# zihang-student/Codes-of-IPD-SsN-AMG-method

Measured on AMD Instinct MI355X. Metric: V-cycle throughput (DoF*cycles/sec), m=n=1024 OT grid, higher is better.
Workload: dtype f64

## Files before the change

### codes_of_ipd_ssn_amg_method_amd/csrc/ipd_resident.h

```cpp
#pragma once

#include "ipd_resident_proto.h"

static constexpr int RES_P3_LD = 1152;
static constexpr int RES_P4_LD = 2 * RES_P4_SEG + 64;

struct ResLevelDesc {
    int N, nf, S;
    const unsigned short* pci;
    const double* pva;
    const double* diag;
    const double* dinv;
    const double* Axi;
    const double* xx;
};
struct ResDesc {
    ResLevelDesc L1, L2;
    ResLevelDesc L3;
    ResCsr Pt2, P2;
    ResCsr Pt3, P3;
    ResCsr Pt4, P4;
    ResCsr A3;
    ResCsr A4;
    int three;
// ... 86 lines not shown
        s1 = __builtin_fma(a[q + 1], y[q + 1], s1);
        s2 = __builtin_fma(a[q + 2], y[q + 2], s2);
        s3 = __builtin_fma(a[q + 3], y[q + 3], s3);
    }
    return (s0 + s1) + (s2 + s3);
}

__device__ __forceinline__ double res_csr_rowdot(const ResCsr& M, int e0, int e1, int lane,
                                                 const double* sm, int off) {
    double s = 0.0;
    for (int t = e0 + lane; t < e1; t += 64 * 8) {
        int jj[8];
        double aa[8];
#pragma unroll
        for (int u = 0; u < 8; ++u) {
            const int tt = t + 64 * u;
            const int tc = tt < e1 ? tt : e0;
            jj[u] = M.ci[tc];
            aa[u] = M.va[tc];
        }
#pragma unroll
        for (int u = 0; u < 8; ++u) s += (t + 64 * u < e1) ? aa[u] * sm[off + jj[u]] : 0.0;
    }
    return wave_sum(s);
}

__device__ __forceinline__ double res_red8(const double* red) {
    double t = 0.0;
#pragma unroll
    for (int k = 0; k < RES_WAVES; ++k) t += red[k];
    return t;
}

__device__ __forceinline__ double res_red8_tree(const double* red) {
    static_assert(RES_WAVES == 8, "eight waves");
    double v[RES_WAVES];
#pragma unroll
    for (int k = 0; k < RES_WAVES; ++k) v[k] = red[k];
    return ((v[0] + v[1]) + (v[2] + v[3])) + ((v[4] + v[5]) + (v[6] + v[7]));
}

__device__ __forceinline__ void res_swap_halves32(double& a, double& b) {
    const auto lo = __builtin_amdgcn_permlane32_swap((unsigned)__double2loint(a), (unsigned)__double2loint(b), false, false);
    const auto hi = __builtin_amdgcn_permlane32_swap((unsigned)__double2hiint(a), (unsigned)__double2hiint(b), false, false);
    a = __hiloint2double((int)hi[0], (int)lo[0]);
    b = __hiloint2double((int)hi[1], (int)lo[1]);
}
__device__ __forceinline__ void res_swap_rows16(double& a, double& b) {
    const auto lo = __builtin_amdgcn_permlane16_swap((unsigned)__double2loint(a), (unsigned)__double2loint(b), false, false);
    const auto hi = __builtin_amdgcn_permlane16_swap((unsigned)__double2hiint(a), (unsigned)__double2hiint(b), false, false);
    a = __hiloint2double((int)hi[0], (int)lo[0]);
    b = __hiloint2double((int)hi[1], (int)lo[1]);
}
__device__ __forceinline__ void res_cs_rows(const double (&A)[RES_WAVES][2], double v0, double v1, double* part_out,
                                            int w, int lane) {
    static_assert(RES_WAVES == 8, "eight rows per block and workgroup");
    double p[RES_WAVES];
#pragma unroll
    for (int r = 0; r < RES_WAVES; ++r) p[r] = __builtin_fma(A[r][1], v1, A[r][0] * v0);
    double q[4];
#pragma unroll
    for (int k = 0; k < 4; ++k) {
        res_swap_halves32(p[k], p[k + 4]);
        q[k] = p[k] + p[k + 4];
    }
    double t[2];
#pragma unroll
    for (int k = 0; k < 2; ++k) {
        res_swap_rows16(q[k], q[k + 2]);
        t[k] = q[k] + q[k + 2];
    }
    const bool f = (lane & 8) != 0;
    const double keep = f ? t[1] : t[0], send = f ? t[0] : t[1];
    double u = keep + dpp_get<0x128, 0xf>(send);
    u = subwave_sum(u, 8);
    if ((lane & 7) == 0) part_out[8 * (lane >> 3) + w] = u;
}

enum res_class {
    RES_CL_HALF = 0,
    RES_CL_START = 1,
    RES_CL_RR = 2,
    RES_CL_RESTRICT = 3,
    RES_CL_LEVEL2 = 4,
    RES_CL_PROLONG = 5,
    RES_CL_TOP = 6,
    RES_NCLASS = 8
};

template <int KE1, int KE2, int KE3 = 0, bool POLY2 = false, bool DIAG = true, bool FULL = false>
__global__ __launch_bounds__(BT, 2) void k_resident(const ResDesc D, const double* __restrict__ bvec,
                                                    double* xg, double* out, int fixed_cycles) {
    static_assert(!POLY2 || (KE3 == 0 && KE1 == 16), "POLY2: three-level hierarchies in column slices (resident_takes_poly2)");
    static_assert(!FULL || POLY2, "FULL: the composed instantiation only (resident_takes_full)");
    static_assert(DIAG || KE1 == 16, "the production form exists for the column-slice kernels");
    constexpr int FG = 2 * BT / RES_WAVES;
    if constexpr (FULL) __builtin_assume(__builtin_amdgcn_workitem_id_x() < (unsigned)BT);
    constexpr bool THREE = KE3 > 0;
    constexpr bool POLY3 = KE3 == 1;
    constexpr int K3 = (THREE && !POLY3) ? KE3 : 2;
    extern __shared__ __attribute__((aligned(16))) char res_smem[];
    double* sm = reinterpret_cast<double*>(res_smem);
    const char* smb = res_smem;
    const int tid = threadIdx.x, w = tid >> 6, lane = tid & 63;
#define RES_REMOTE (FULL ? 0 : D.remote)
#define RES_WIDENT (FULL ? 1 : D.wident)
    const int b = blockIdx.x, G = FULL ? FG : gridDim.x - (RES_REMOTE ? 1 : 0);
    const int N1 = FULL ? 4 * BT : D.L1.N, N2 = FULL ? 2 * BT : D.L2.N, nf = FULL ? 2 * BT : D.L1.nf, nc = N1 - nf;
    const int Nt = FULL ? 1 : D.Nt;
    if (RES_REMOTE && b == G) {
        __shared__ PhaseLds tail_lds;
        __shared__ double tail_red[16];
        __shared__ double tail_part[48 + SOLVE_ML + 1];
        __shared__ int tail_stat[RES_WAVES];
        res_tail_workgroup(D.tail, res_smem, &tail_lds, tail_red, tail_part, tail_stat);
        return;
    }
    constexpr int oX = 0, oE1 = RES_NMAX, oE2 = 2 * RES_NMAX, oRR1 = 3 * RES_NMAX;
    constexpr int oR1 = 4 * RES_NMAX, oAX1 = 5 * RES_NMAX, oR2 = 6 * RES_NMAX, oRR2 = 7 * RES_NMAX;
    constexpr int oAX2 = 8 * RES_NMAX;
    constexpr int oRHO = 9 * RES_NMAX;
    constexpr int oBETA = oAX2 + RES_NMAX / 2;
    constexpr int oU = oRR2;
    constexpr int oR3 = 9 * RES_NMAX + RES_NMAX / 2, oE3 = oR3 + RES_TAIL_MAX, oP3 = oE3 + RES_TAIL_MAX;
    constexpr int oPART = oR3, oPART9 = oR3 + 2 * RES_WAVES * RES_WAVES;
    static_assert(2 * RES_WAVES * RES_WAVES + 2 * RES_WAVES <= 3 * RES_TAIL_MAX, "the totals fit the tail's slots");
    constexpr int oRED = oP3 + RES_TAIL_MAX;
    constexpr int oPUB = oRED + 2 * RES_WAVES;
    constexpr int oOWN = oPUB + 2 * RES_WAVES;
// ... 143 lines not shown
#define dgC sm[oOWN + 3 * RES_WAVES + w]
#define dvC sm[oOWN + 4 * RES_WAVES + w]
#define bC sm[oOWN + 5 * RES_WAVES + w]
#define dg2 sm[oOWN + 6 * RES_WAVES + w]
#define dv2 sm[oOWN + 7 * RES_WAVES + w]
#define dg3 sm[oOWN + 8 * RES_WAVES + w]
#define dv3 sm[oOWN + 9 * RES_WAVES + w]
    const bool nsp = FULL ? true : D.isnsp != 0;
    const double xx1 = nsp ? D.L1.xx[0] : 1.0, xx2 = nsp ? D.L2.xx[0] : 1.0;
    const double xx3 = (THREE && nsp) ? D.L3.xx[0] : 1.0;
    const double rxx1 = 1.0 / xx1, rxx2 = 1.0 / xx2, rxx3 = 1.0 / xx3;
    for (int j = tid; j < N1; j += BT) {
        sm[oX + j] = xg[j];
        sm[oE1 + j] = 0.0;
        sm[oAX1 + j] = D.L1.Axi[j];
    }
    for (int j = tid; j < N2; j += BT) {
        sm[oE2 + j] = 0.0;
        sm[oAX2 + j] = D.L2.Axi[j];
    }
    if (THREE)
        for (int j = tid; j < N3; j += BT) {
            sm[oE3L + j] = 0.0;
            sm[oAX3L + j] = D.L3.Axi[j];
        }
    const bool tail1 = FULL ? true : !THREE && Nt == 1 && N2 <= RES_NMAX / 2;
    constexpr int oP3C = oRR2 + RES_NMAX / 2;
    const bool lfirst = FULL ? true : D.localfirst && D.nu >= 1 && N2 <= RES_NMAX / 2 && nf <= RES_NMAX / 2;
    const bool lfirst2 = lfirst && !THREE;
    constexpr int oDV1 = oR2 + RES_NMAX / 2, oDV2 = oE2 + RES_NMAX / 2;
    if (lfirst) {
        for (int j = tid; j < nf; j += BT) sm[oDV1 + j] = D.L1.dinv[j];
        if (lfirst2)
            for (int j = tid; j < N2; j += BT) sm[oDV2 + j] = D.L2.dinv[j];
    }
    const bool xm = FULL ? true : !THREE && D.xm != 0 && nc == N2 && D.wident != 0;
    unsigned xbits = 0;
    if (xm) {
        unsigned long long wf[16], wc[16];
#pragma unroll
        for (int q = 0; q < 16; ++q) {
            wf[q] = D.xm_fbits[(size_t)rF * D.xm_nwf + (q < D.xm_nwf ? q : 0)];
            wc[q] = D.xm_cbits[(size_t)(rC - nf) * D.xm_nwc + (q < D.xm_nwc ? q : 0)];
        }
        unsigned lo = 0, hi = 0;
#pragma unroll
        for (int q = 0; q < 16; ++q) {
            lo |= (vF && q < D.xm_nwf) ? (unsigned)((wf[q] >> lane) & 1ull) << q : 0u;
            hi |= (vC && q < D.xm_nwc) ? (unsigned)((wc[q] >> lane) & 1ull) << q : 0u;
        }
        xbits = lo | (hi << 16);
        for (int j = tid; j < nf; j += BT) sm[oRHO + j] = D.xm_rho[j];
        for (int j = tid; j < nc; j += BT) sm[oBETA + j] = D.xm_beta[j];
    }
    double h33 = 0.0;
    if (tail1) {
        for (int j = tid; j < N2; j += BT) {
            double v = 0.0;
            if (POLY2) {
                v = D.p2rows[(size_t)N2 * D.p2ld + j];
            } else {
                for (int t = D.P3.rp[j]; t < D.P3.rp[j + 1]; ++t)
                    if (D.P3.ci[t] == 0) v = D.P3.va[t];
            }
            sm[oP3C + j] = v;
        }
        for (int t = D.A3.rp[0]; t < D.A3.rp[1]; ++t)
            if (D.A3.ci[t] == 0) h33 = D.A3.va[t];
    }
    if (tid == 0) *fail = 0;
    __syncthreads();

    const auto rs = __builtin_amdgcn_make_buffer_rsrc(D.gran0, 0, 2 * RES_GRAN_MAX * 16, 0x00020000);
    unsigned seq = 0;
    bool dead = false;
    const bool dbg = DIAG && D.dbg != nullptr && b == 0 && tid == 0;
#define RES_SKIPPED(sq) (DIAG && (sq) == D.dbg_skip_seq && b == G - 1)
    if (dbg) {
        dbg_acc[0] = dbg_acc[3] = dbg_acc[4] = dbg_acc[5] = dbg_acc[6] = dbg_acc[7] = dbg_acc[8] = 0;
        dbg_acc[1] = __builtin_amdgcn_s_memtime();
        dbg_acc[2] = __builtin_amdgcn_s_memrealtime();
        if constexpr (KE1 == 16)
            for (int k = 0; k < 2 * RES_NCLASS; ++k) cls_acc[k] = 0u;
    }
    auto cls_begin = [&](int c) __attribute__((always_inline)) {
        if constexpr (KE1 == 16) {
            if (dbg) __hip_atomic_fetch_sub(cls_acc + c, (unsigned)__builtin_amdgcn_s_memtime(), __ATOMIC_RELAXED, __HIP_MEMORY_SCOPE_WORKGROUP);
        }
    };
    auto cls_end = [&](int c) __attribute__((always_inline)) {
        if constexpr (KE1 == 16) {
            if (dbg) {
                __hip_atomic_fetch_add(cls_acc + c, (unsigned)__builtin_amdgcn_s_memtime(), __ATOMIC_RELAXED, __HIP_MEMORY_SCOPE_WORKGROUP);
                __hip_atomic_fetch_add(cls_acc + RES_NCLASS + c, 1u, __ATOMIC_RELAXED, __HIP_MEMORY_SCOPE_WORKGROUP);
            }
        }
    };

#define RES_HANDOFF(NJ, n, gA, cA, gB, cB, STORE, EXTRA, want_sums, t0, t1)                        \
    RES_HANDOFF_P(NJ, n, gA, cA, gB, cB, {}, STORE, EXTRA, want_sums, t0, t1)
#define RES_HANDOFF_P(NJ, n, gA, cA, gB, cB, PRE, STORE, EXTRA, want_sums, t0, t1)                 \
    RES_HANDOFF_PV(NJ, n, gA, cA, gB, cB, sm[oPUB + lane], PRE, STORE, EXTRA, want_sums, t0, t1)
#define RES_HANDOFF_PV(NJ, n, gA, cA, gB, cB, PUBV, PRE, STORE, EXTRA, want_sums, t0, t1)          \
    RES_HANDOFF_PVA(NJ, n, gA, cA, gB, cB, PUBV, PRE, STORE, {}, EXTRA, want_sums, t0, t1)
#define RES_HANDOFF_PVA(NJ, n, gA, cA, gB, cB, PUBV, PRE, STORE, AFTER, EXTRA, want_sums, t0, t1)  \
    do {                                                                                           \
// ... 12 lines not shown
            const bool second_ = lane >= RES_WAVES;                                                \
            if (lane < 2 * RES_WAVES && l8_ < (second_ ? (cB) : (cA)) &&                           \
                !RES_SKIPPED(seq))                                                                 \
                res_publish(rs, seq, (second_ ? (gB) : (gA)) + l8_, (PUBV));                       \
        }                                                                                          \
        double p0 = 0.0, p1 = 0.0;                                                                 \
        _Pragma("unroll") for (int u_ = 0; u_ < NJ; ++u_) {                                        \
            const int j = tid + u_ * BT;                                                           \
            if (j < (n)) { PRE; }                                                                  \
        }                                                                                          \
        EXTRA;                                                                                     \
        if (dbg) dbg_acc[0] -= __builtin_amdgcn_s_memtime();                                       \
        for (int ps_ = 0; ps_ < D.presleep; ++ps_) __builtin_amdgcn_s_sleep(1);                    \
        if (res_sweep<NJ>(rs, seq, (n), dead, D.tmo, hv_, D.pollsleep)) {                             \
            *fail = 1;                                                                             \
            if (lane == 0) __hip_atomic_store(D.tmo, seq, __ATOMIC_RELAXED, __HIP_MEMORY_SCOPE_AGENT); \
        }                                                                                          \
        if (dbg) {                                                                                 \
            const long long t_ = __builtin_amdgcn_s_memtime();                                     \
            dbg_acc[0] += t_;                                                                      \
            dbg_acc[4] -= t_;                                                                      \
        }                                                                                          \
        _Pragma("unroll") for (int u_ = 0; u_ < NJ; ++u_) {                                        \
            const int j = tid + u_ * BT;                                                           \
            if (j < (n)) {                                                                         \
                const double v = hv_[u_];                                                          \
                STORE;                                                                             \
            }                                                                                      \
        }                                                                                          \
        AFTER;                                                                                     \
        if (want_sums) {                                                                           \
            p0 = wave_sum(p0);                                                                     \
            if ((want_sums) > 1) p1 = wave_sum(p1);                                                \
            if (lane == 0) {                                                                       \
                red[w] = p0;                                                                       \
                if ((want_sums) > 1) red[RES_WAVES + w] = p1;                                      \
            }                                                                                      \
        }                                                                                          \
        if (dbg) {                                                                                 \
            const long long t_ = __builtin_amdgcn_s_memtime();                                     \
            dbg_acc[4] += t_;                                                                      \
            dbg_acc[5] -= t_;                                                                      \
        }                                                                                          \
        __syncthreads();                                                                           \
        if (dbg) dbg_acc[5] += __builtin_amdgcn_s_memtime();                                       \
        if (want_sums) {                                                                           \
            t0 = res_red8_tree(red);                                                               \
            if ((want_sums) > 1) t1 = res_red8_tree(red + RES_WAVES);                              \
        }                                                                                          \
    } while (0)

    auto masked_sum = [&](unsigned bits, int off, int n) __attribute__((always_inline)) {
        double s0 = 0.0, s1 = 0.0;
        (void)n;
        const double* base = sm + off + lane;
        for (int q0 = 0; q0 < 16; q0 += 8) {
            double x[8];
#pragma unroll
            for (int q = 0; q < 8; ++q) x[q] = base[64 * (q0 + q)];
            const unsigned bq = bits >> q0;
#pragma unroll
            for (int q = 0; q < 8; q += 2) {
                s0 += ((bq >> q) & 1u) ? x[q] : 0.0;
                s1 += ((bq >> (q + 1)) & 1u) ? x[q + 1] : 0.0;
            }
        }
        return wave_sum(s0 + s1);
    };
    double c1 = 0.0, c2s = 0.0;
    double sumr2p = 0.0;
    (void)sumr2p;
    const double p2ws = POLY2 ? D.p2w[N2] : 0.0;
    double dum0 = 0.0, dum1 = 0.0;
    (void)dum0;
    (void)dum1;

    int csFed = -1, csBuf = 0;
    double eFo = 0.0, eCo = 0.0;
    (void)csFed; (void)csBuf; (void)eFo; (void)eCo;
    bool topfed = false;
    (void)topfed;
    auto cs_both_rows = [&](int off) __attribute__((always_inline)) {
        const double f0 = tid < nc ? sm[off + nf + tid] : 0.0, f1 = tid + BT < nc ? sm[off + nf + tid + BT] : 0.0;
        const double g0 = tid < nf ? sm[off + tid] : 0.0, g1 = tid + BT < nf ? sm[off + tid + BT] : 0.0;
        res_cs_rows(AF, f0, f1, sm + oPART, w, lane);
        res_cs_rows(AC, g0, g1, sm + oPART + RES_WAVES * RES_WAVES, w, lane);
        csFed = -1;
        eFo = eCo = 0.0;
    };

    auto cs_row_value = [&](int off, bool rhs_b) __attribute__((always_inline)) {
        const bool sec = lane >= RES_WAVES;
        const int r = lane & (RES_WAVES - 1);
        const int row = sec ? RES_OWN_ROW(loC, hiC, r) : RES_OWN_ROW(loF, hiF, r);
        const double T = res_red8_tree(sm + oPART + RES_WAVES * lane);
        const double dg_ = sm[oOWN + (sec ? 3 : 0) * RES_WAVES + r];
        const double base = rhs_b ? sm[oOWN + (sec ? 5 : 2) * RES_WAVES + r] : sm[oR1 + row];
        return base - (T + dg_ * sm[off + row]);
    };

    auto top = [&]() __attribute__((always_inline)) {
        double nrm2 = 0.0, sumr = 0.0;
        bool fed = false;
        if constexpr (FULL) {
            if (topfed) {
                fed = true;
                topfed = false;
                ++seq;
                if (*fail) dead = true;
                double hv[4];
                if (dbg) dbg_acc[0] -= __builtin_amdgcn_s_memtime();
                for (int ps = 0; ps < D.presleep; ++ps) __builtin_amdgcn_s_sleep(1);
                if (res_sweep<4>(rs, seq, N1, dead, D.tmo, hv, D.pollsleep)) {
                    *fail = 1;
                    if (lane == 0) __hip_atomic_store(D.tmo, seq, __ATOMIC_RELAXED, __HIP_MEMORY_SCOPE_AGENT);
                }
                if (dbg) {
                    const long long t_ = __builtin_amdgcn_s_memtime();
                    dbg_acc[0] += t_;
                    dbg_acc[4] -= t_;
                }
                double p0 = 0.0, p1 = 0.0;
#pragma unroll
                for (int u = 0; u < 4; ++u) {
                    const int j = tid + u * BT;
                    const double v = hv[u];
                    sm[oR1 + j] = v;
                    sm[oE1 + j] = 0.0;
                    p0 += v * v;
                    p1 += v;
                }
                p0 = wave_sum(p0);
// ... 129 lines not shown
                    const long long t_ = __builtin_amdgcn_s_memtime();
                    dbg_acc[0] += t_;
                    dbg_acc[4] -= t_;
                }
#pragma unroll
                for (int u = 0; u < 2; ++u) {
                    const int j = blk0 + tid + u * BT;
                    const double en = hv[u] + cc;
                    sm[oE1 + j] = en;
                    if (frows) {
                        const double xn = xo[u] + en;
                        sm[oX + j] = xn;
                        mv[u] = xn;
                    } else {
                        mv[u] = en;
                    }
                }
                csBuf ^= 1;
                if (frows)
                    res_cs_rows(AC, mv[0], mv[1], sm + oPART + RES_WAVES * RES_WAVES * csBuf, w, lane);
                else
                    res_cs_rows(AF, mv[0], mv[1], sm + oPART + RES_WAVES * RES_WAVES * csBuf, w, lane);
                if (dbg) {
                    const long long t_ = __builtin_amdgcn_s_memtime();
                    dbg_acc[4] += t_;
                    dbg_acc[3] -= t_;
                }
                __syncthreads();
                if (dbg) dbg_acc[3] += __builtin_amdgcn_s_memtime();
                cls_end(RES_CL_HALF);
                cls_begin(frows ? RES_CL_TOP : RES_CL_RR);
                const double* totF = frows ? sm + oPART3 : sm + oPART + RES_WAVES * RES_WAVES * csBuf;
                const double* totC = frows ? sm + oPART + RES_WAVES * RES_WAVES * csBuf : sm + oPART3;
                if (frows) {
                    if (w == 0 && lane < 2 * RES_WAVES) {
                        const bool sec = lane >= RES_WAVES;
                        const int r = lane & (RES_WAVES - 1);
                        const int row = (sec ? loC : loF) + r;
                        const double T = res_red8_tree((sec ? totC : totF) + RES_WAVES * r);
                        const double dg_ = sm[oOWN + (sec ? 3 : 0) * RES_WAVES + r];
                        const double base = sm[oOWN + (sec ? 5 : 2) * RES_WAVES + r];
                        const double val = base - (T + dg_ * sm[oX + row]);
                        if (!RES_SKIPPED(seq + 1)) res_publish(rs, seq + 1, row, val);
                    }
                    topfed = true;
                } else {
                    if (w == 0 && lane < RES_WAVES) {
                        const double TF = res_red8_tree(totF + RES_WAVES * lane);
                        const double TC = res_red8_tree(totC + RES_WAVES * lane);
                        const double dF_ = sm[oOWN + 0 * RES_WAVES + lane], dC_ = sm[oOWN + 3 * RES_WAVES + lane];
                        const double rF_ = sm[oR1 + loF + lane], rC_ = sm[oR1 + loC + lane];
                        const double val = rF_ - (TF + dF_ * eFo);
                        if (!RES_SKIPPED(seq + 1)) res_publish(rs, seq + 1, loF + lane, val);
                        sm[oRR1 + loC + lane] = rC_ - (TC + dC_ * eCo);
                    }
                }
                csFed = -1;
                eFo = eCo = 0.0;
                return;
            }
        }
        cls_begin(start ? RES_CL_START : RES_CL_HALF);
        ++seq;
        if (*fail) dead = true;
        if (ezero && first) {
            eFo = eCo = 0.0;
            cs_finish(frows, first, true, seq);
        } else if (!FULL && csFed != me) {
            const double v0 = tid < noth ? sm[oE1 + oth0 + tid] : 0.0;
            const double v1 = tid + BT < noth ? sm[oE1 + oth0 + tid + BT] : 0.0;
            csBuf ^= 1;
            if (frows)
                res_cs_rows(AF, v0, v1, sm + oPART + RES_WAVES * RES_WAVES * csBuf, w, lane);
            else
                res_cs_rows(AC, v0, v1, sm + oPART + RES_WAVES * RES_WAVES * csBuf, w, lane);
            eFo = sm[oE1 + RES_OWN_ROW(loF, hiF, lane)];
            eCo = sm[oE1 + RES_OWN_ROW(loC, hiC, lane)];
            __syncthreads();
            cs_finish(frows, first, false, seq);
        }
        const double cc = c1;
        double pa[2] = {0.0, 0.0}, pb[2] = {0.0, 0.0}, p0 = 0.0;
        if (!first) {
#pragma unroll
            for (int u = 0; u < 2; ++u) {
                const int j = tid + u * BT;
                if (j < nblk) {
                    pa[u] = sm[oR1 + blk0 + j];
                    pb[u] = sm[oAX1 + blk0 + j];
                }
            }
            for (int jo = tid; jo < noth; jo += BT) {
                const double en = sm[oE1 + oth0 + jo] + cc;
                sm[oE1 + oth0 + jo] = en;
                p0 += sm[oR1 + oth0 + jo] - sm[oAX1 + oth0 + jo] * en;
            }
        }
        if (dbg) dbg_acc[0] -= __builtin_amdgcn_s_memtime();
        for (int ps = 0; ps < D.presleep; ++ps) __builtin_amdgcn_s_sleep(1);
        double hv[2] = {0.0, 0.0};
        if (res_sweep<2>(rs, seq, nblk, dead, D.tmo, hv, D.pollsleep)) {
            *fail = 1;
            if (lane == 0) __hip_atomic_store(D.tmo, seq, __ATOMIC_RELAXED, __HIP_MEMORY_SCOPE_AGENT);
        }
        if (dbg) {
            const long long t_ = __builtin_amdgcn_s_memtime();
            dbg_acc[0] += t_;
// ... 387 lines not shown
            {
                const double s = wave_sum(res_rowdot<K3, 8 * oE3L>(c3, a3, smb)) + dg3 * sm[oE3L + r3];
                if (lane == 0) sm[oPUB + w] = sm[oR3L + r3] - s;
                RES_HANDOFF3({ sm[oRR3L + j] = v; }, 0, dum0);
            }
            if (RES_REMOTE)
                remote_tail(D.Pt4, oRR3L, oE3L, oR3L, oAX3L, xx3, N3, c3s);
            else
                local_tail(D.Pt4, D.A4, D.P4, oRR3L, oE3L, oR3L, oAX3L, xx3, N3, c3s);
            for (int s = 0; s < nu; ++s) sweep3(false);
        }
    };

    auto visit2 = [&](bool keep) __attribute__((always_inline)) {
        const int nu = D.nu;
        for (int s = (lfirst2 && !keep) ? 1 : 0; s < nu; ++s) sweep2(!keep && s == 0);
        {
            cls_begin(RES_CL_LEVEL2);
            const double s = wave_sum(res_rowdot_fma<KE2, 8 * oE2>(c2, a2, smb)) + dg2 * sm[oE2 + r2];
            if (lane == 0) sm[oPUB + w] = sm[oR2 + r2] - s;
            RES_HANDOFF(4, N2, lo2, hi2 - lo2, 0, 0, { sm[oRR2 + j] = v; }, {}, 0, dum0, dum1);
        }
        if (dbg) dbg_acc[7] -= __builtin_amdgcn_s_memtime();
        if (THREE) {
            {
                const double s = res_csr_rowdot(D.Pt3, rowp[12 * w + 8], rowp[12 * w + 9], lane, sm, oRR2);
                if (lane == 0) sm[oPUB + w] = s;
                double sumr = 0.0;
                RES_HANDOFF3({ sm[oR3L + j] = v; sm[oE3L + j] = 0.0; p0 += v; }, (nsp ? 1 : 0), sumr);
                c3s = nsp ? sumr * rxx3 : 0.0;
                sumr3 = sumr;
            }
            for (int leg = 0; leg < (D.wcycle ? 2 : 1); ++leg) visit3(leg == 1);
            {
                const double sP = res_csr_rowdot(D.P3, rowp[12 * w + 10], rowp[12 * w + 11], lane, sm, oE3L);
                if (lane == 0) sm[oPUB + w] = sm[oE2 + r2] + sP;
                double xig = 0.0;
                RES_HANDOFF_P(4, N2, lo2, hi2 - lo2, 0, 0, { pa_[u_] = sm[oR2 + j]; pb_[u_] = sm[oAX2 + j]; },
                              { sm[oE2 + j] = v; p0 += pa_[u_] - pb_[u_] * v; }, {}, (nsp ? 1 : 0), xig, dum1);
                c2s = nsp ? xig * rxx2 : 0.0;
            }
        } else {
            tail();
        }
        if (dbg) dbg_acc[7] += __builtin_amdgcn_s_memtime();
        cls_end(RES_CL_LEVEL2);
        for (int s = 0; s < nu; ++s) sweep2(false);
    };

    auto poly2_fed = [&]() __attribute__((always_inline)) {
        if constexpr (POLY2) {
            ++seq;
            if (*fail) dead = true;
            if (dbg) dbg_acc[3] -= __builtin_amdgcn_s_memtime();
            __syncthreads();
            if (dbg) dbg_acc[3] += __builtin_amdgcn_s_memtime();
            const bool pub = w == 0 && lane < RES_WAVES && lane < hi2 - lo2;
            if (pub && !RES_SKIPPED(seq)) res_publish(rs, seq, lo2 + lane, sm[oPUB + lane]);
            const double s0 = tid < N2 ? sm[oP3C + tid] : 0.0, s1 = tid + BT < N2 ? sm[oP3C + tid + BT] : 0.0;
            double hv[2] = {0.0, 0.0};
            if (dbg) dbg_acc[0] -= __builtin_amdgcn_s_memtime();
            for (int ps = 0; ps < D.presleep; ++ps) __builtin_amdgcn_s_sleep(1);
            if (res_sweep<2>(rs, seq, N2, dead, D.tmo, hv, D.pollsleep)) {
                *fail = 1;
                if (lane == 0) __hip_atomic_store(D.tmo, seq, __ATOMIC_RELAXED, __HIP_MEMORY_SCOPE_AGENT);
            }
            if (dbg) {
                const long long t_ = __builtin_amdgcn_s_memtime();
                dbg_acc[0] += t_;
                dbg_acc[4] -= t_;
            }
            const double v0 = tid < N2 ? hv[0] : 0.0, v1 = tid + BT < N2 ? hv[1] : 0.0;
            res_cs_rows(B2, v0, v1, sm + oPART, w, lane);
            const double ps = wave_sum(s0 * v0 + s1 * v1);
            const double p1 = nsp ? wave_sum(v0 + v1) : 0.0;
            if (lane == 0) {
                red[w] = ps;
                red[RES_WAVES + w] = p1;
            }
            if (dbg) {
                const long long t_ = __builtin_amdgcn_s_memtime();
                dbg_acc[4] += t_;
                dbg_acc[3] -= t_;
            }
            __syncthreads();
            if (dbg) dbg_acc[3] += __builtin_amdgcn_s_memtime();
            cls_end(RES_CL_RESTRICT);
            cls_begin(RES_CL_LEVEL2);
            ++seq;
            if (*fail) dead = true;
            if (w == 0 && lane < RES_WAVES) {
                const double wB = sm[oOWN + 6 * RES_WAVES + lane], mp = sm[oOWN + 7 * RES_WAVES + lane];
                const double T = res_red8_tree(sm + oPART + RES_WAVES * lane);
                const double sr = res_red8_tree(red), sum1 = res_red8_tree(red + RES_WAVES);
                const double d = res_pcg_1x1(sr + p2ws * sum1, h33, D.pcg_maxit);
                const double val = T + wB * sum1 + mp * d;
                if (pub && !RES_SKIPPED(seq)) res_publish(rs, seq, lo2 + lane, val);
            }
            double be[2] = {0.0, 0.0};
            (void)be;
            if constexpr (FULL) {
                be[0] = sm[oBETA + tid];
                be[1] = sm[oBETA + tid + BT];
            }
            if (dbg) dbg_acc[0] -= __builtin_amdgcn_s_memtime();
            for (int ps = 0; ps < D.presleep; ++ps) __builtin_amdgcn_s_sleep(1);
            if (res_sweep<2>(rs, seq, N2, dead, D.tmo, hv, D.pollsleep)) {
                *fail = 1;
                if (lane == 0) __hip_atomic_store(D.tmo, seq, __ATOMIC_RELAXED, __HIP_MEMORY_SCOPE_AGENT);
            }
            if (dbg) {
                const long long t_ = __builtin_amdgcn_s_memtime();
                dbg_acc[0] += t_;
                dbg_acc[4] -= t_;
            }
            if (tid < N2) sm[oE2 + tid] = hv[0];
            if (tid + BT < N2) sm[oE2 + tid + BT] = hv[1];
            if constexpr (FULL) {
                sm[oU + tid] = be[0] * hv[0];
                sm[oU + tid + BT] = be[1] * hv[1];
            }
            if (dbg) {
                const long long t_ = __builtin_amdgcn_s_memtime();
                dbg_acc[4] += t_;
                dbg_acc[5] -= t_;
            }
            __syncthreads();
            if (dbg) dbg_acc[5] += __builtin_amdgcn_s_memtime();
            cls_end(RES_CL_LEVEL2);
        }
    };

    auto cycle = [&]() __attribute__((always_inline)) {
        const int nu = D.nu;
        if constexpr (FULL) cs_finish(false, false, false, seq + 1);
        for (int s = 0; s < nu; ++s) sweep1(false, s == 0, s == nu - 1, s == 0);
        if constexpr (FULL) {
            ++seq;
            if (*fail) dead = true;
            const double rh0 = sm[oRHO + tid], rh1 = sm[oRHO + tid + BT];
            double hv[2] = {0.0, 0.0};
            if (dbg) dbg_acc[0] -= __builtin_amdgcn_s_memtime();
            for (int ps = 0; ps < D.presleep; ++ps) __builtin_amdgcn_s_sleep(1);
            if (res_sweep<2>(rs, seq, nf, dead, D.tmo, hv, D.pollsleep)) {
                *fail = 1;
                if (lane == 0) __hip_atomic_store(D.tmo, seq, __ATOMIC_RELAXED, __HIP_MEMORY_SCOPE_AGENT);
            }
            if (dbg) {
                const long long t_ = __builtin_amdgcn_s_memtime();
                dbg_acc[0] += t_;
                dbg_acc[4] -= t_;
            }
            sm[oRR1 + tid] = hv[0] * rh0;
            sm[oRR1 + tid + BT] = hv[1] * rh1;
            if (dbg) {
                const long long t_ = __builtin_amdgcn_s_memtime();
                dbg_acc[4] += t_;
                dbg_acc[5] -= t_;
            }
            __syncthreads();
            if (dbg) dbg_acc[5] += __builtin_amdgcn_s_memtime();
        } else
        {
            if constexpr (CS1) {
                cls_begin(RES_CL_RR);
                cs_both_rows(oE1);
            } else {
            const double sF = wave_sum(res_rowdot_fma<KR1, 8 * oE1>(cF, aF, smb)) + dgF * sm[oE1 + rF];
            const double sC = wave_sum(res_rowdot_fma<KR1, 8 * oE1>(cC, aC, smb)) + dgC * sm[oE1 + rC];
            if (lane == 0) {
                sm[oPUB + w] = sm[oR1 + rF] - sF;
                sm[oPUB + RES_WAVES + w] = sm[oR1 + rC] - sC;
            }
            }
            if constexpr (CS1) {
                if (xm) {
                    RES_HANDOFF_PV(4, N1, loF, hiF - loF, loC, hiC - loC, cs_row_value(oE1, false),
                                   { pa_[u_] = j < nf ? sm[oRHO + j] : 1.0; },
                                   { sm[oRR1 + j] = j < nf ? v * pa_[u_] : v; }, {}, 0, dum0, dum1);
                } else {
                    RES_HANDOFF_PV(4, N1, loF, hiF - loF, loC, hiC - loC, cs_row_value(oE1, false), {},
                                   { sm[oRR1 + j] = v; }, {}, 0, dum0, dum1);
                }
            } else
            if (xm) {
                RES_HANDOFF_P(4, N1, loF, hiF - loF, loC, hiC - loC, { pa_[u_] = j < nf ? sm[oRHO + j] : 1.0; },
                              { sm[oRR1 + j] = j < nf ? v * pa_[u_] : v; }, {}, 0, dum0, dum1);
            } else {
                RES_HANDOFF(4, N1, loF, hiF - loF, loC, hiC - loC, { sm[oRR1 + j] = v; }, {}, 0, dum0, dum1);
            }
        }
        {
            cls_end(RES_CL_RR);
            cls_begin(RES_CL_RESTRICT);
            if (dbg) dbg_acc[6] -= __builtin_amdgcn_s_memtime();
            const double s = xm ? sm[oBETA + r2] * masked_sum(xbits >> 16, oRR1, nf) + sm[oRR1 + rC]
                                : res_csr_rowdot(D.Pt2, rowp[12 * w + 0], rowp[12 * w + 1], lane, sm, oRR1) +
                                      (RES_WIDENT ? sm[oRR1 + rC] : 0.0);
            if (dbg) dbg_acc[6] += __builtin_amdgcn_s_memtime();
            if (lane == 0) sm[oPUB + w] = s;
            if constexpr (POLY2) {
                poly2_fed();
            } else {
            double sumr = 0.0;
            RES_HANDOFF(4, N2, lo2, hi2 - lo2, 0, 0, { sm[oR2 + j] = v; sm[oE2 + j] = 0.0; p0 += v; }, {},
                        (nsp ? 1 : 0), sumr, dum1);
            c2s = nsp ? sumr * rxx2 : 0.0;
            sumr2p = sumr;
            if (lfirst2 && !POLY2) {
                const double cc = c2s;
                double p0 = 0.0;
                for (int j = tid; j < N2; j += BT) {
                    const double g_i = sm[oR2 + j] - sm[oAX2 + j] * cc;
                    const double en = sm[oDV2 + j] * g_i + cc;
                    sm[oE2 + j] = en;
                    p0 += sm[oR2 + j] - sm[oAX2 + j] * en;
                }
                if (nsp) {
                    p0 = wave_sum(p0);
                    if (lane == 0) red[w] = p0;
                }
                __syncthreads();
                if (nsp) c2s = res_red8(red) / xx2;
                __syncthreads();
            }
            cls_end(RES_CL_RESTRICT);
            }
        }
        if constexpr (!POLY2)
            for (int leg = 0; leg < (D.wcycle ? 2 : 1); ++leg) visit2(leg == 1);
        {
            cls_begin(RES_CL_PROLONG);
            if (dbg) dbg_acc[6] -= __builtin_amdgcn_s_memtime();
            if constexpr (FULL) {
                const double sF = sm[oRHO + rF] * masked_sum(xbits & 0xffffu, oU, N2);
                if (dbg) dbg_acc[6] += __builtin_amdgcn_s_memtime();
                if (lane == 0) sm[oPUB + w] = sm[oE1 + rF] + sF;
                ++seq;
                if (*fail) dead = true;
                if (dbg) dbg_acc[3] -= __builtin_amdgcn_s_memtime();
                __syncthreads();
                if (dbg) dbg_acc[3] += __builtin_amdgcn_s_memtime();
                if (w == 0 && lane < RES_WAVES && !RES_SKIPPED(seq)) res_publish(rs, seq, loF + lane, sm[oPUB + lane]);
                double pa[2], pb[2], tc[2], hv[2] = {0.0, 0.0};
#pragma unroll
                for (int u = 0; u < 2; ++u) {
                    const int j = tid + u * BT;
                    pa[u] = sm[oR1 + j];
                    pb[u] = sm[oAX1 + j];
                    const double ec = sm[oE1 + nf + j] + sm[oE2 + j];
                    sm[oE1 + nf + j] = ec;
                    tc[u] = sm[oR1 + nf + j] - sm[oAX1 + nf + j] * ec;
                }
                if (dbg) dbg_acc[0] -= __builtin_amdgcn_s_memtime();
                for (int ps = 0; ps < D.presleep; ++ps) __builtin_amdgcn_s_sleep(1);
                if (res_sweep<2>(rs, seq, nf, dead, D.tmo, hv, D.pollsleep)) {
                    *fail = 1;
                    if (lane == 0) __hip_atomic_store(D.tmo, seq, __ATOMIC_RELAXED, __HIP_MEMORY_SCOPE_AGENT);
                }
                if (dbg) {
                    const long long t_ = __builtin_amdgcn_s_memtime();
                    dbg_acc[0] += t_;
                    dbg_acc[4] -= t_;
                }
                double p0 = 0.0;
#pragma unroll
                for (int u = 0; u < 2; ++u) {
                    sm[oE1 + tid + u * BT] = hv[u];
                    p0 += pa[u] - pb[u] * hv[u];
                }
                p0 += tc[0];
                p0 += tc[1];
                csBuf ^= 1;
                res_cs_rows(AC, hv[0], hv[1], sm + oPART + RES_WAVES * RES_WAVES * csBuf, w, lane);
                p0 = wave_sum(p0);
                if (lane == 0) red[w] = p0;
                if (dbg) {
                    const long long t_ = __builtin_amdgcn_s_memtime();
                    dbg_acc[4] += t_;
                    dbg_acc[5] -= t_;
                }
                __syncthreads();
                if (dbg) dbg_acc[5] += __builtin_amdgcn_s_memtime();
                c1 = res_red8_tree(red) * rxx1;
                eFo = sm[oE1 + loF + (lane & (RES_WAVES - 1))];
                eCo = sm[oE1 + loC + (lane & (RES_WAVES - 1))];
                cs_finish(false, true, false, seq + 1);
                csFed = 1;
                cls_end(RES_CL_PROLONG);
            } else {
            if (xm) {
                for (int j = tid; j < N2; j += BT) sm[oU + j] = sm[oBETA + j] * sm[oE2 + j];
                __syncthreads();
            }
            const double sF = xm ? sm[oRHO + rF] * masked_sum(xbits & 0xffffu, oU, N2)
                                 : res_csr_rowdot(D.P2, rowp[12 * w + 2], rowp[12 * w + 3], lane, sm, oE2);
// ... 104 lines not shown
```

### codes_of_ipd_ssn_amg_method_amd/csrc/ipd_resident_host.hip

```cpp
#include "ipd_cycle_state.h"

#include <chrono>
#include <condition_variable>
#include <mutex>

#include "ipd_resident_big.h"

struct ResidentState {
    bool ok = false;
    bool off = false;
    ResidentPlan plan;
    ResDesc desc{};
    ResBigDesc big{};
    unsigned skip_publish = 0;
    unsigned char* block = nullptr;
    size_t block_bytes = 0;
    double* out = nullptr;
    int timeouts = 0;
    long long last_handoffs = 0;
    int last_cycles = 0;
    bool last_full = false, last_diag = false;
    int capacity = -1;
    int line_ke = 0, line_ke3 = 0;
    bool mask_form() const { return plan.kind == RESIDENT_BIG || plan.kind == RESIDENT_DEEP; }
// ... 147 lines not shown
                       (const unsigned long long*)mo.fbits, mo.nwf, mo.alpha, mo.beta, mo.diag, h->L[2].P.rp,
                       h->L[2].P.ci, h->L[2].P.va, rho, bad);
    IPD_KERNEL_CHECK();
    return ctx->fetch1(bad) == 0 ? rho : nullptr;
}

static ResCsr res_csr(const Csr& m) { return ResCsr{m.rp, m.ci, m.va}; }
static ResLevelDesc res_level(const LevelDev& d) {
    return ResLevelDesc{d.N, d.nf, d.S, d.pci, d.pva, d.diag, d.dinv, d.Axi, d.xx};
}

template <class Desc>
static void set_cycle_options(Desc& D, const ipd_amg* h, int presleep) {
    D.nu = h->opts.smoth;
    D.isnsp = h->opts.isnsp;
    D.wcycle = h->opts.cycle == 'w';
    D.anycycle = (h->opts.cycle == 'w' || h->opts.cycle == 'v');
    D.maxit = h->opts.maxit;
    D.retol = h->opts.retol;
    D.pcg_maxit = h->opts.pcg_maxit;
    D.pollsleep = 1;
    D.presleep = presleep;
    D.dbg_skip_seq = 0;
}

static unsigned char* alloc_resident_block(ipd_amg* h, ResidentState& R, ResTail& T, unsigned*& tmo, size_t gran_bytes,
                                           bool tail) {
    const size_t tbytes = (size_t)RES_GRAN_MAX * 16;
    R.block_bytes = gran_bytes + 16 + (tail ? 4 * tbytes + 16 : 0);
    R.block = reinterpret_cast<unsigned char*>(h->arena->alloc_bytes(R.block_bytes));
    tmo = T.tmo = reinterpret_cast<unsigned*>(R.block + gran_bytes);
    T.tin = tail ? R.block + gran_bytes + 16 : R.block;
    T.tout = tail ? R.block + gran_bytes + 16 + 2 * tbytes : R.block;
    T.tctl = tail ? reinterpret_cast<unsigned*>(R.block + gran_bytes + 16 + 4 * tbytes) : T.tmo;
    return R.block;
}

static BPolyPack pack_resident_poly(ipd_amg* h, CycleState* st, int k, int seg, int ld) {
    const BPolyPack pb = pack_bpoly(h->ctx, h, st, k, h->opts.isnsp, 0, true, seg, ld);
    record_rows_op(st, h, k, pb);
    st->level_forms.resize((size_t)h->J + 1, 0);
    st->level_forms[(size_t)k] |= 64;
    return pb;
}

static void commit_resident(ipd_amg* h, ResidentState& R, const ResidentPlan& p, const PlanSwitches& sw) {
    R.plan = p;
    R.capacity = -1;
    R.skip_publish = sw.res_skip_publish;
    if (!R.out) R.out = h->arena->alloc<double>(4 + 2 * ((size_t)std::max(h->opts.maxit, 0) + 2));
    R.ok = true;
}

static void choose_full_shape(const ipd_amg* h, const CycleState* st, ResidentState& R, const PlanSwitches& sw) {
    if (!R.ok || R.plan.kind != RESIDENT_K) return;
    const std::vector<LevelShape> shapes = level_shapes(h, st);
    const ResDesc& D = R.desc;
    const ResidentFullFacts facts{D.xm != 0, D.wident, D.isnsp, D.localfirst != 0};
    const bool full = resident_takes_full(R.plan, resident_inputs(h, st, shapes), facts, sw);
    if (full != R.plan.key.full) {
        R.plan.key.full = full;
        R.capacity = -1;
    }
}

void prepare_resident(ipd_amg* h, CycleState* st, const std::vector<LevelShape>& shapes, const PlanSwitches& sw) {
    st->res = std::make_shared<ResidentState>();
    ResidentState& R = *st->res;
    R.off = sw.no_resident;
    const ResidentPlan p = plan_resident(resident_inputs(h, st, shapes), sw);
    if (p.considered && switch_on("IPD_DEBUG_LEVELS"))
        std::fprintf(stderr, "[ipd] resident plan: J=%d nf=%d nc=%d S1=%d S2=%d S3=%d N4=%d Nt=%d k_sub=%d sub_lds=%zu\n", h->J,
                     h->L[1].nf, h->L[1].A.nr - h->L[1].nf, p.S[1], p.S[2], st->run[3].dev.S,
                     h->J >= 4 ? h->L[4].A.nr : 0, h->L[3].A.nr, st->k_sub, st->img[IMG_SUB].lds);
    if (p.kind == RESIDENT_NONE) return;
    const Level& l1 = h->L[1];
    const Level& l2 = h->L[2];
    const Level& l3 = h->L[3];
    const int N2 = l2.A.nr, nf = l1.nf;
    ResDesc D{};
    D.L1 = res_level(resident_rows(h, st, p, 1));
    D.L2 = res_level(resident_rows(h, st, p, 2));
    D.Pt2 = res_csr(l2.Pt);
    D.P2 = res_csr(l2.P);
    D.Pt3 = res_csr(l3.Pt);
    D.P3 = res_csr(l3.P);
    D.A3 = res_csr(l3.A);
    D.Nt = p.Nin;
    D.three = p.three ? 1 : 0;
    D.A4 = res_csr(p.three ? h->L[4].A : l3.A);
    if (p.three) {
        if (p.poly3) {
            const BPolyPack pb = pack_resident_poly(h, st, 3, 512, RES_P3_LD);
            D.p3rows = pb.M;
            D.p3w = pb.W;
            if (p.poly4) {
                const BPolyPack pb4 = pack_resident_poly(h, st, 4, RES_P4_SEG, RES_P4_LD);
                D.p4rows = pb4.M;
                D.p4w = pb4.W;
                D.N5 = h->L[5].A.nr;
            }
        }
        D.L3 = res_level(resident_rows(h, st, p, 3));
        D.Pt4 = res_csr(h->L[4].Pt);
        D.P4 = res_csr(h->L[4].P);
    } else {
        D.L3 = D.L2;
        D.Pt4 = res_csr(l3.Pt);
        D.P4 = res_csr(l3.P);
    }
    set_cycle_options(D, h, sw.res_presleep >= 0 ? sw.res_presleep : 8);
    D.wident = p.wident > 0 ? 1 : 0;
    if (p.wident < 0) {
        int* bad = zeroed<int>(h->ctx, 1);
        hipLaunchKernelGGL(k_res_check_ident, dim3(cdiv(N2, 256)), dim3(256), 0, h->ctx->stream, nf, N2,
                           res_csr(l2.P), res_csr(l2.Pt), bad);
        IPD_KERNEL_CHECK();
        D.wident = h->ctx->fetch1(bad) == 0 ? 1 : 0;
    }
    D.localfirst = 1;
    const size_t gbytes = (size_t)RES_GRAN_MAX * 16;
    D.gran0 = alloc_resident_block(h, R, D.tail, D.tmo, 2 * gbytes, p.remote);
    D.gran1 = D.gran0 + gbytes;
    D.remote = p.remote ? 1 : 0;
    ResTail& T = D.tail;
    T.sub = resident_image(st, p.tail_image);
    T.root = p.tail_root;
    T.nin = p.tail_root == 5 ? D.N5 : D.Nt;
    T.nout = p.tail_root == 3 ? D.L2.N : D.L3.N;
    T.answer_root = D.p3rows != nullptr;
    T.Pout = p.tail_root == 3 ? D.P3 : D.P4;
    T.wcycle = D.wcycle;
    T.tail_bm = p.tail_bm ? 1 : 0;
    R.desc = D;
    R.line_ke = p.key.ke;
    R.line_ke3 = p.key.ke3;
    commit_resident(h, R, p, sw);
}

struct ResidentSlots {
    std::mutex mu;
    std::condition_variable cv;
    int used[64] = {0};
    bool acquire(int device, int workgroups, int cus, int wait_ms) {
        std::unique_lock<std::mutex> lock(mu);
        if (workgroups > cus) return false;
        const bool got = cv.wait_for(lock, std::chrono::milliseconds(wait_ms),
                                     [&] { return used[device & 63] + workgroups <= cus; });
        if (!got) return false;
        used[device & 63] += workgroups;
        return true;
    }
    void release(int device, int workgroups) {
        {
            std::lock_guard<std::mutex> lock(mu);
            used[device & 63] -= workgroups;
        }
        cv.notify_all();
    }
};
static ResidentSlots& resident_slots() {
    static ResidentSlots s;
    return s;
}
// ... 350 lines not shown
```

Baseline: 58.10 million.

## Replace shared-memory masked transfer sums with per-wave butterfly partials in FULL path

In the FULL resident kernel, restriction and prolongation transfers no longer write per-column vectors to shared memory and then have each wave do a masked row sum after a barrier. Each wave now preloads its slice of the coarse and fine mask bits and reduces its own columns into per-row partials with a permlane/DPP butterfly. The partials go into double-buffered shared slots and are summed by the publishing lanes. This removes one block barrier and a shared round trip per transfer, and the presleep default is raised for the FULL variant. The cost is extra register pressure and more intricate buffer-parity bookkeeping.

```diff
diff --git a/codes_of_ipd_ssn_amg_method_amd/csrc/ipd_resident.h b/codes_of_ipd_ssn_amg_method_amd/csrc/ipd_resident.h
--- a/codes_of_ipd_ssn_amg_method_amd/csrc/ipd_resident.h
+++ b/codes_of_ipd_ssn_amg_method_amd/csrc/ipd_resident.h
@@ -162,12 +162,8 @@
     a = __hiloint2double((int)hi[0], (int)lo[0]);
     b = __hiloint2double((int)hi[1], (int)lo[1]);
 }
-__device__ __forceinline__ void res_cs_rows(const double (&A)[RES_WAVES][2], double v0, double v1, double* part_out,
-                                            int w, int lane) {
+__device__ __forceinline__ double res_cs_butterfly(double (&p)[RES_WAVES], int lane) {
     static_assert(RES_WAVES == 8, "eight rows per block and workgroup");
-    double p[RES_WAVES];
-#pragma unroll
-    for (int r = 0; r < RES_WAVES; ++r) p[r] = __builtin_fma(A[r][1], v1, A[r][0] * v0);
     double q[4];
 #pragma unroll
     for (int k = 0; k < 4; ++k) {
@@ -183,8 +179,36 @@
     const bool f = (lane & 8) != 0;
     const double keep = f ? t[1] : t[0], send = f ? t[0] : t[1];
     double u = keep + dpp_get<0x128, 0xf>(send);
-    u = subwave_sum(u, 8);
+    return subwave_sum(u, 8);
+}
+__device__ __forceinline__ void res_cs_totals(double (&p)[RES_WAVES], double* part_out, int w, int lane) {
+    const double u = res_cs_butterfly(p, lane);
     if ((lane & 7) == 0) part_out[8 * (lane >> 3) + w] = u;
+}
+__device__ __forceinline__ void res_cs_rows(const double (&A)[RES_WAVES][2], double v0, double v1, double* part_out,
+                                            int w, int lane) {
+    double p[RES_WAVES];
+#pragma unroll
+    for (int r = 0; r < RES_WAVES; ++r) p[r] = __builtin_fma(A[r][1], v1, A[r][0] * v0);
+    res_cs_totals(p, part_out, w, lane);
+}
+
+__device__ __forceinline__ void res_xfer_parts(unsigned bits2, double y0, double y1, double (&a)[RES_WAVES]) {
+#pragma unroll
+    for (int r = 0; r < RES_WAVES; ++r) {
+        const double z0 = ((bits2 >> (2 * r)) & 1u) ? y0 : 0.0, z1 = ((bits2 >> (2 * r + 1)) & 1u) ? y1 : 0.0;
+        a[r] = z0 + z1;
+    }
+}
+__device__ __forceinline__ double res_xfer_row_sum(double (&a)[RES_WAVES], int lane) {
+    double t = res_cs_butterfly(a, lane);
+    t = t + dpp_get<0x128, 0xf>(t);
+    double t0 = t, t1 = t;
+    res_swap_rows16(t0, t1);
+    t = t0 + t1;
+    t0 = t1 = t;
+    res_swap_halves32(t0, t1);
+    return t0 + t1;
 }
 
 enum res_class {
@@ -434,6 +458,26 @@
         xbits = lo | (hi << 16);
         for (int j = tid; j < nf; j += BT) sm[oRHO + j] = D.xm_rho[j];
         for (int j = tid; j < nc; j += BT) sm[oBETA + j] = D.xm_beta[j];
+    }
+    unsigned xslice = 0;
+    (void)xslice;
+    if constexpr (FULL) {
+        static_assert(BT == 64 * RES_WAVES, "a wave's 64 columns are one word of a mask row");
+        unsigned long long wc[RES_WAVES][2], wf[RES_WAVES][2];
+#pragma unroll
+        for (int r = 0; r < RES_WAVES; ++r)
+#pragma unroll
+            for (int u = 0; u < 2; ++u) {
+                wc[r][u] = D.xm_cbits[(size_t)(lo2 + r) * (2 * RES_WAVES) + w + RES_WAVES * u];
+                wf[r][u] = D.xm_fbits[(size_t)(loF + r) * (2 * RES_WAVES) + w + RES_WAVES * u];
+            }
+#pragma unroll
+        for (int r = 0; r < RES_WAVES; ++r)
+#pragma unroll
+            for (int u = 0; u < 2; ++u) {
+                xslice |= (unsigned)((wc[r][u] >> lane) & 1ull) << (2 * r + u);
+                xslice |= (unsigned)((wf[r][u] >> lane) & 1ull) << (16 + 2 * r + u);
+            }
     }
     double h33 = 0.0;
     if (tail1) {
@@ -552,8 +596,28 @@
 
     auto masked_sum = [&](unsigned bits, int off, int n) __attribute__((always_inline)) {
         double s0 = 0.0, s1 = 0.0;
+        (void)s0; (void)s1;
         (void)n;
         const double* base = sm + off + lane;
+        if constexpr (KE1 == 16) {
+            double a[RES_WAVES];
+#pragma unroll
+            for (int q0 = 0; q0 < 8; q0 += 4) {
+                double x[8];
+#pragma unroll
+                for (int q = 0; q < 4; ++q) {
+                    x[q] = base[64 * (q0 + q)];
+                    x[4 + q] = base[64 * (q0 + q + 8)];
+                }
+#pragma unroll
+                for (int q = 0; q < 4; ++q) {
+                    const double z0 = ((bits >> (q0 + q)) & 1u) ? x[q] : 0.0;
+                    const double z1 = ((bits >> (q0 + q + 8)) & 1u) ? x[4 + q] : 0.0;
+                    a[q0 + q] = z0 + z1;
+                }
+            }
+            return res_xfer_row_sum(a, lane);
+        } else {
         for (int q0 = 0; q0 < 16; q0 += 8) {
             double x[8];
 #pragma unroll
@@ -566,6 +630,7 @@
             }
         }
         return wave_sum(s0 + s1);
+        }
     };
     double c1 = 0.0, c2s = 0.0;
     double sumr2p = 0.0;
@@ -578,6 +643,8 @@
     int csFed = -1, csBuf = 0;
     double eFo = 0.0, eCo = 0.0;
     (void)csFed; (void)csBuf; (void)eFo; (void)eCo;
+    double rrCo = 0.0;
+    (void)rrCo;
     bool topfed = false;
     (void)topfed;
     auto cs_both_rows = [&](int off) __attribute__((always_inline)) {
@@ -813,7 +880,7 @@
                         const double rF_ = sm[oR1 + loF + lane], rC_ = sm[oR1 + loC + lane];
                         const double val = rF_ - (TF + dF_ * eFo);
                         if (!RES_SKIPPED(seq + 1)) res_publish(rs, seq + 1, loF + lane, val);
-                        sm[oRR1 + loC + lane] = rC_ - (TC + dC_ * eCo);
+                        rrCo = rC_ - (TC + dC_ * eCo);
                     }
                 }
                 csFed = -1;
@@ -1307,11 +1374,20 @@
         if constexpr (POLY2) {
             ++seq;
             if (*fail) dead = true;
+            const bool pub = w == 0 && lane < RES_WAVES && lane < hi2 - lo2;
+            if constexpr (FULL) {
+                if (pub) {
+                    const double be_ = sm[oBETA + lo2 + lane];
+                    const double T = res_red8_tree(sm + oPART + RES_WAVES * RES_WAVES * csBuf + RES_WAVES * lane);
+                    const double val = be_ * T + rrCo;
+                    if (!RES_SKIPPED(seq)) res_publish(rs, seq, lo2 + lane, val);
+                }
+            } else {
             if (dbg) dbg_acc[3] -= __builtin_amdgcn_s_memtime();
             __syncthreads();
             if (dbg) dbg_acc[3] += __builtin_amdgcn_s_memtime();
-            const bool pub = w == 0 && lane < RES_WAVES && lane < hi2 - lo2;
             if (pub && !RES_SKIPPED(seq)) res_publish(rs, seq, lo2 + lane, sm[oPUB + lane]);
+            }
             const double s0 = tid < N2 ? sm[oP3C + tid] : 0.0, s1 = tid + BT < N2 ? sm[oP3C + tid + BT] : 0.0;
             double hv[2] = {0.0, 0.0};
             if (dbg) dbg_acc[0] -= __builtin_amdgcn_s_memtime();
@@ -1326,7 +1402,9 @@
                 dbg_acc[4] -= t_;
             }
             const double v0 = tid < N2 ? hv[0] : 0.0, v1 = tid + BT < N2 ? hv[1] : 0.0;
-            res_cs_rows(B2, v0, v1, sm + oPART, w, lane);
+            if constexpr (FULL) csBuf ^= 1;
+            double* part2 = sm + oPART + (FULL ? RES_WAVES * RES_WAVES * csBuf : 0);
+            res_cs_rows(B2, v0, v1, part2, w, lane);
             const double ps = wave_sum(s0 * v0 + s1 * v1);
             const double p1 = nsp ? wave_sum(v0 + v1) : 0.0;
             if (lane == 0) {
@@ -1346,7 +1424,7 @@
             if (*fail) dead = true;
             if (w == 0 && lane < RES_WAVES) {
                 const double wB = sm[oOWN + 6 * RES_WAVES + lane], mp = sm[oOWN + 7 * RES_WAVES + lane];
-                const double T = res_red8_tree(sm + oPART + RES_WAVES * lane);
+                const double T = res_red8_tree(part2 + RES_WAVES * lane);
                 const double sr = res_red8_tree(red), sum1 = res_red8_tree(red + RES_WAVES);
                 const double d = res_pcg_1x1(sr + p2ws * sum1, h33, D.pcg_maxit);
                 const double val = T + wB * sum1 + mp * d;
@@ -1372,8 +1450,10 @@
             if (tid < N2) sm[oE2 + tid] = hv[0];
             if (tid + BT < N2) sm[oE2 + tid + BT] = hv[1];
             if constexpr (FULL) {
-                sm[oU + tid] = be[0] * hv[0];
-                sm[oU + tid + BT] = be[1] * hv[1];
+                double a[RES_WAVES];
+                res_xfer_parts(xslice >> 16, be[0] * hv[0], be[1] * hv[1], a);
+                csBuf ^= 1;
+                res_cs_totals(a, sm + oPART + RES_WAVES * RES_WAVES * csBuf, w, lane);
             }
             if (dbg) {
                 const long long t_ = __builtin_amdgcn_s_memtime();
@@ -1406,8 +1486,12 @@
                 dbg_acc[0] += t_;
                 dbg_acc[4] -= t_;
             }
-            sm[oRR1 + tid] = hv[0] * rh0;
-            sm[oRR1 + tid + BT] = hv[1] * rh1;
+            {
+                double a[RES_WAVES];
+                res_xfer_parts(xslice & 0xffffu, hv[0] * rh0, hv[1] * rh1, a);
+                csBuf ^= 1;
+                res_cs_totals(a, sm + oPART + RES_WAVES * RES_WAVES * csBuf, w, lane);
+            }
             if (dbg) {
                 const long long t_ = __builtin_amdgcn_s_memtime();
                 dbg_acc[4] += t_;
@@ -1448,12 +1532,14 @@
         {
             cls_end(RES_CL_RR);
             cls_begin(RES_CL_RESTRICT);
+            if constexpr (!FULL) {
             if (dbg) dbg_acc[6] -= __builtin_amdgcn_s_memtime();
             const double s = xm ? sm[oBETA + r2] * masked_sum(xbits >> 16, oRR1, nf) + sm[oRR1 + rC]
                                 : res_csr_rowdot(D.Pt2, rowp[12 * w + 0], rowp[12 * w + 1], lane, sm, oRR1) +
                                       (RES_WIDENT ? sm[oRR1 + rC] : 0.0);
             if (dbg) dbg_acc[6] += __builtin_amdgcn_s_memtime();
             if (lane == 0) sm[oPUB + w] = s;
+            }
             if constexpr (POLY2) {
                 poly2_fed();
             } else {
@@ -1486,17 +1572,16 @@
             for (int leg = 0; leg < (D.wcycle ? 2 : 1); ++leg) visit2(leg == 1);
         {
             cls_begin(RES_CL_PROLONG);
-            if (dbg) dbg_acc[6] -= __builtin_amdgcn_s_memtime();
+            if (!FULL && dbg) dbg_acc[6] -= __builtin_amdgcn_s_memtime();
             if constexpr (FULL) {
-                const double sF = sm[oRHO + rF] * masked_sum(xbits & 0xffffu, oU, N2);
-                if (dbg) dbg_acc[6] += __builtin_amdgcn_s_memtime();
-                if (lane == 0) sm[oPUB + w] = sm[oE1 + rF] + sF;
                 ++seq;
                 if (*fail) dead = true;
-                if (dbg) dbg_acc[3] -= __builtin_amdgcn_s_memtime();
-                __syncthreads();
-                if (dbg) dbg_acc[3] += __builtin_amdgcn_s_memtime();
-                if (w == 0 && lane < RES_WAVES && !RES_SKIPPED(seq)) res_publish(rs, seq, loF + lane, sm[oPUB + lane]);
+                if (w == 0 && lane < RES_WAVES) {
+                    const double e_own = sm[oE1 + loF + lane], rh_ = sm[oRHO + loF + lane];
+                    const double T = res_red8_tree(sm + oPART + RES_WAVES * RES_WAVES * csBuf + RES_WAVES * lane);
+                    const double sF = rh_ * T;
+                    if (!RES_SKIPPED(seq)) res_publish(rs, seq, loF + lane, e_own + sF);
+                }
                 double pa[2], pb[2], tc[2], hv[2] = {0.0, 0.0};
 #pragma unroll
                 for (int u = 0; u < 2; ++u) {
diff --git a/codes_of_ipd_ssn_amg_method_amd/csrc/ipd_resident_host.hip b/codes_of_ipd_ssn_amg_method_amd/csrc/ipd_resident_host.hip
--- a/codes_of_ipd_ssn_amg_method_amd/csrc/ipd_resident_host.hip
+++ b/codes_of_ipd_ssn_amg_method_amd/csrc/ipd_resident_host.hip
@@ -223,6 +223,8 @@
     R.ok = true;
 }
 
+static constexpr int RES_PRESLEEP = 8, RES_PRESLEEP_FULL = 11;
+
 static void choose_full_shape(const ipd_amg* h, const CycleState* st, ResidentState& R, const PlanSwitches& sw) {
     if (!R.ok || R.plan.kind != RESIDENT_K) return;
     const std::vector<LevelShape> shapes = level_shapes(h, st);
@@ -233,6 +235,7 @@
         R.plan.key.full = full;
         R.capacity = -1;
     }
+    R.desc.presleep = sw.res_presleep >= 0 ? sw.res_presleep : full ? RES_PRESLEEP_FULL : RES_PRESLEEP;
 }
 
 void prepare_resident(ipd_amg* h, CycleState* st, const std::vector<LevelShape>& shapes, const PlanSwitches& sw) {
@@ -280,7 +283,7 @@
         D.Pt4 = res_csr(l3.Pt);
         D.P4 = res_csr(l3.P);
     }
-    set_cycle_options(D, h, sw.res_presleep >= 0 ? sw.res_presleep : 8);
+    set_cycle_options(D, h, sw.res_presleep >= 0 ? sw.res_presleep : RES_PRESLEEP);
     D.wident = p.wident > 0 ? 1 : 0;
     if (p.wident < 0) {
         int* bad = zeroed<int>(h->ctx, 1);
```

Result: slower. 57.42 million (-1.2%).
